# hjmkt/wrenc

Measured on AMD Instinct MI355X. Metric: all-intra encode fps at fixed QP (CTU RD search + final pass); bit-exactness vs the CPU oracle is checked in `parity`, higher is better.
Workload: dtype u8/i16/i32 (+i64 trellis costs, f32 RD cost)

## Files before the change

include/wrenc_gpu.h:

```cpp
#ifndef WRENC_GPU_H
#define WRENC_GPU_H

#include <stddef.h>
#include <stdint.h>

#ifdef __cplusplus
extern "C" {
#endif

typedef struct wrenc_gpu_ctx wrenc_gpu_ctx;

enum wrenc_gpu_status {
    WRENC_GPU_OK = 0,
    WRENC_GPU_EINVAL = -1,
    WRENC_GPU_ENODEV = -2,
    WRENC_GPU_ENOMEM = -3,
    WRENC_GPU_EHIP = -4,
    WRENC_GPU_ESTATE = -5,
    WRENC_GPU_ELEVEL = -6
};

typedef struct wrenc_gpu_config {
    int32_t width;
    int32_t height;
// ... 113 lines not shown
int wrenc_gpu_test_avail_tab(wrenc_gpu_ctx* ctx, int* differences);

int wrenc_gpu_stats_enable(wrenc_gpu_ctx* ctx, int on);

int wrenc_gpu_last_encode_stats(wrenc_gpu_ctx* ctx, float* total_ms, float* kernel_ms_sum,
                                int* n_launches);
typedef struct wrenc_gpu_kernel_stats {
    float ms_sum;
    int32_t launches;
    int64_t ctu_pictures;
} wrenc_gpu_kernel_stats;
int wrenc_gpu_last_encode_kernel_stats(wrenc_gpu_ctx* ctx, wrenc_gpu_kernel_stats out[2]);

int wrenc_gpu_final_pass_mismatches(wrenc_gpu_ctx* ctx, long long* count);

int wrenc_gpu_test_fwd_dct(wrenc_gpu_ctx* ctx, const int16_t* res, int log2n, int count,
                           int16_t* coef);
int wrenc_gpu_test_fwd_dct32(wrenc_gpu_ctx* ctx, const int16_t* res, int count, int16_t* coef,
                             int use_mfma, int reps, float* kernel_ms);
int wrenc_gpu_test_inv_dct32(wrenc_gpu_ctx* ctx, const int16_t* deq, int count, int16_t* res,
                             int use_mfma, int reps, float* kernel_ms);
int wrenc_gpu_test_quantize_pk(wrenc_gpu_ctx* ctx, const int16_t* coef, int log2n, int nc, int n_packs, int16_t* levels,
                               int64_t* level_cost);
int wrenc_gpu_test_inv_dct(wrenc_gpu_ctx* ctx, const int16_t* deq, int log2n, int count,
                           int16_t* res);
int wrenc_gpu_test_quantize(wrenc_gpu_ctx* ctx, const int16_t* coef, int log2n, int count,
                            int16_t* levels, int64_t* level_cost);
int wrenc_gpu_test_quantize_p16(wrenc_gpu_ctx* ctx, const int16_t* coef, int count, int16_t* levels,
                                int64_t* level_cost);
int wrenc_gpu_test_dequantize(wrenc_gpu_ctx* ctx, const int16_t* levels, int log2n, int count,
                              int16_t* deq);
int wrenc_gpu_test_fwd_dct4_reg(wrenc_gpu_ctx* ctx, const int16_t* res, int count, int16_t* coef);
int wrenc_gpu_test_inv_dct4_reg(wrenc_gpu_ctx* ctx, const int16_t* levels, int count, int16_t* res);

int wrenc_gpu_test_predict(wrenc_gpu_ctx* ctx, const uint8_t* rec_y, const uint8_t* rec_cb,
                           const uint8_t* rec_cr, int n_items, const int32_t* items, uint8_t* out,
                           size_t out_bytes);

#ifdef __cplusplus
}
#endif
#endif
```

wrenc_amd/csrc/dev_predict.h:

```cpp
#pragma once

namespace wrenc {

__device__ __forceinline__ int pdpc_w(int n_scale, int i) {
    const int sh = (i << 1) >> n_scale;
    return sh > 5 ? 0 : (32 >> sh);
}

__device__ __forceinline__ void build_refs(Ctx c, int comp, int tx, int ty, int tlg) {
#ifdef WRENC_EXP_SKIP_REFS
    return;
#endif
    c = uni(c);
    comp = uni(comp);
    tx = uni(tx);
    ty = uni(ty);
    tlg = uni(tlg);
    const int cs = comp ? 1 : 0;
    const int nb = comp ? 2 : 1;
    const int n = 1 << (tlg - cs);
    const int tn = 1 << tlg;
    const int cx = tx >> cs, cy = ty >> cs;
    const int st = 1 << cs;
    const int avm = block_avail_mask(c, tx, ty, tlg, st);
// ... 221 lines not shown
}
__device__ __forceinline__ void stage_org(const Ctx& c, int comps, int tx, int ty, int tlg, int lbyte = kOrgStage,
                                          int cword = 256) {
    uint32_t* dst = (uint32_t*)((char*)SH.r2 + lbyte);
#ifdef WRENC_EXP_NO_ORG
    for (int w = LANE; w < 384; w += 64) dst[w] = 0x50607080u + (uint32_t)w;
    WSYNC();
    return;
#endif
    if (comps & 1) {
        const int words = 1 << (2 * tlg - 2);
        for (int w = LANE; w < words; w += 64) {
            const int row = (4 * w) >> tlg, col = (4 * w) & ((1 << tlg) - 1);
            dst[w] = *(const GLOBAL_AS uint32_t*)&c.org[(ty + row) * 32 + tx + col];
        }
    }
    if (comps & 2) {
        const int lg = tlg - 1;
        const int words = 1 << (2 * lg - 2);
        for (int w = LANE; w < 2 * words; w += 64) {
            const int pl = w >= words ? 1 : 0;
            const int ww = w - pl * words;
            const int row = (4 * ww) >> lg, col = (4 * ww) & ((1 << lg) - 1);
            dst[cword + w] = *(const GLOBAL_AS uint32_t*)&c.org[1024 + pl * 256 + ((ty >> 1) + row) * 16 + (tx >> 1) + col];
        }
    }
    WSYNC();
}

__device__ __forceinline__ void stage_org_leaf(const Ctx& c, int comps, int tx, int ty, int tlg) {
    stage_org(c, comps, tx, ty, tlg, kOrgLeaf, 64);
}

enum { PRED_SCRATCH = 0, PRED_TILE = 1, PRED_PARK = 2, PRED_PARK16 = 3 };
constexpr int kParkByte = 160;
static_assert(kParkByte >= 144 && kParkByte % 16 == 0 && kParkByte + 288 <= 448, "Lds::decw: decisions of an 8x8 pack | its park | the server's results");
__device__ __forceinline__ uint8_t* park16(int i, int nl) {
    if (i < nl) return (uint8_t*)SH.r1 + 1536 + i;
    const int j = i - nl;
    return j < 128 ? (uint8_t*)SH.r2 + 1536 + j : (uint8_t*)SH.decw + 384 + (j - 128);
}
template <bool full>
__device__ __forceinline__ int emit_sample(const Ctx& c, int o, int i, int v, int pc, int x, int y, int to_tile, int nl = 0) {
    const int d = o - v;
    if (full) {
        SH.r1[i] = (int16_t)d;
        if (to_tile == PRED_TILE)
            rec_put(pc, x, y, v);
        else if (to_tile == PRED_PARK)
            ((uint8_t*)SH.decw)[kParkByte + i] = (uint8_t)v;
        else if (to_tile == PRED_PARK16)
            *park16(i, nl) = (uint8_t)v;
        else
            c.pred_scratch[i] = (uint8_t)v;
    }
    return d < 0 ? -d : d;
}

template <bool full>
__device__ __forceinline__ int predict(Ctx c, int comp, int tx, int ty, int tlg, int mode, int rbase = 0,
                                       int to_tile = PRED_TILE, int nl = 0, CclmPick pick = CclmPick{}) {
#ifdef WRENC_EXP_SKIP_PRED
    return 0;
#endif
    c = uni(c);
    rbase = uni(rbase);
    to_tile = uni(to_tile);
    nl = uni(nl);
    comp = uni(comp);
    tx = uni(tx);
    ty = uni(ty);
    tlg = uni(tlg);
    mode = uni(mode);
    const int cs = comp ? 1 : 0;
    const int nb = comp ? 2 : 1;
    const int lg = tlg - cs;
    const int n = 1 << lg;
    const int cx = tx >> cs, cy = ty >> cs;
    const int nn = n * n;
    const int obyte = org_byte(comp, tlg);
    const bool olds = tlg <= 4;
    int sad = 0;
    if (mode >= LT_CCLM) {
        CclmPick cp = pick;
        if (!pick.have) cp = cclm_pick(cclm_params(c, tx, ty, tlg, mode), 0);
        const int a0 = cp.a0, a1 = cp.a1, k0 = cp.k0, k1 = cp.k1, b0 = cp.b0, b1 = cp.b1;
        const bool flat128 = cp.flat128, avail_l = cp.avail_l;
// ... 589 lines not shown
```

wrenc_amd/csrc/dev_quant.h:

```cpp
#pragma once

namespace wrenc {

__device__ __forceinline__ long long ldq_at(Ctx c, int bits) {
    return bits < 256 ? (long long)SHT.ldq[bits] : c.k->ldq[bits];
}
__device__ __forceinline__ long long lv_at(Ctx c, int a) {
    return a < 256 ? (long long)SHT.lv[a] : c.k->lv[a];
}
template <int CTRL>
__device__ __forceinline__ int dpp_quad(int v) {
    return __builtin_amdgcn_mov_dpp(v, CTRL, 0xF, 0xF, true);
}

struct DecMasks {
    uint32_t m01, m23;
};
__device__ __forceinline__ DecMasks dec_masks(const uint16_t* dec16, int p) {
    const uint2 v = *(const uint2*)(dec16 + (p >> 4) * 4);
    DecMasks m;
    m.m01 = v.x;
    m.m23 = v.y;
    return m;
}
// ... 489 lines not shown
    unsigned zmask = 0;
    int fnz = P;
    int level = 0;
    if (mine) {
        int state = entry;
        level = (int16_t)emit_level(c, tc, qd, p == P - 1, nib, p, 0, state, zmask, sum_nz, fnz, ovf);
    }
    level = __builtin_amdgcn_ds_permute(4 * at, level);
    const int pf = row_min_i32(fnz);
    if (mine && (zmask & 1u) && p > pf) sum_nz += SHT.lv[0];
    {
        const long long hi = sum_nz >> 24;
        const int ra = row_sum_i32((int)(sum_nz & 0xFFFFFF)), rb = row_sum_i32((int)(hi & 0xFFFFFF)), rc = row_sum_i32((int)(hi >> 24));
#pragma unroll
        for (int b = 0; b < 4; ++b) {
            const long long a0 = (long long)(unsigned)__builtin_amdgcn_readlane(ra, 16 * b);
            const long long a1 = (long long)(unsigned)__builtin_amdgcn_readlane(rb, 16 * b);
            const long long a2 = (long long)__builtin_amdgcn_readlane(rc, 16 * b);
            lvl[b] = a0 + ((a1 + (a2 << 24)) << 24);
            if (__builtin_amdgcn_readlane(pf, 16 * b) < P) *any_mask |= 1 << b;
        }
    }
    if (__ballot(ovf != 0) != 0ULL) *overflow = 1;
    WSYNC();
    PROF_MARK(q3_);
    PROF_ADD2(PH_QTRACE, q2_, q3_);
    return level;
}
__device__ __forceinline__ int dequantize4_lane(const Ctx& c, int level) {
    constexpr int sh = 8 + 2 - 5 + 1, off = (1 << sh) >> 1;
    const int v = (M24(level, c.k->lsc) + off) >> sh;
    return min(max(v, -32768), 32767);
}


__device__ __forceinline__ void trace_rows64(const Ctx& c, int nblk, const int16_t* tcs, const uint16_t* dec16, int rbase,
                                             const CONST_AS uint16_t* scan, int sh, int off, long long lvl[4], bool any[4], int& ovf,
                                             int start = 0) {
    const int lane = lane_fresh();
    const int row = lane >> 4, i16 = lane & 15;
    const CONST_AS DevConst* k = c.k;
    const int per = start >= 48 ? 1 : (start >= 32 ? 2 : 4);
    const int p0 = start + i16 * per;
    const bool act = row < nblk && p0 < 64;
    const int b = row < nblk ? row : 0;
    const int16_t* btcs = tcs + b * 64;
    const DecMasks dm = dec_masks(dec16 + b * 16, act ? p0 : 0);
    int fmap = kMapId;
    if (act) {
        for (int j = 0; j < per; ++j) {
            const int p = p0 + j;
            const int tc = btcs[p];
            fmap = compose_map(position_map(tc, quotient(k, tc, sh, off), p == 63, dec_nib(dm, p)), fmap);
        }
    }
    int pre = fmap;
    pre = compose_map(pre, __builtin_amdgcn_update_dpp(kMapId, pre, 0x111, 0xF, 0xF, false));
    pre = compose_map(pre, __builtin_amdgcn_update_dpp(kMapId, pre, 0x112, 0xF, 0xF, false));
    pre = compose_map(pre, __builtin_amdgcn_update_dpp(kMapId, pre, 0x114, 0xF, 0xF, false));
    pre = compose_map(pre, __builtin_amdgcn_update_dpp(kMapId, pre, 0x118, 0xF, 0xF, false));
    int entry = __builtin_amdgcn_update_dpp(0, pre, 0x111, 0xF, 0xF, false) & 3;
    if (i16 == 0) entry = 0;
    long long sum_nz = 0;
    unsigned zmask = 0;
    int fnz = 64;
    if (act) {
// ... 419 lines not shown
```

wrenc_amd/csrc/dev_search.h:

```cpp
#pragma once

namespace wrenc {

enum { K_SADLIST = 0, K_FULL = 1, K_NOP = 2, K_SADSEARCH = 3, K_CCLMSEARCH = 4, K_SERVE8 = 5, K_LEAF8 = 7, K_LEAF16 = 8, K_SPLIT8 = 9, K_SERVE4 = 10 };
enum { COPY_NONE = 0, COPY_SAVE = 1, COPY_RESTORE = 2, COPY_PULL = 3 };

#if defined(WRENC_TRACE) || defined(WRENC_EXHAUSTIVE_SPLITS)
constexpr bool kSplitCut = false;
#else
constexpr bool kSplitCut = true;
#endif

#if defined(WRENC_TRACE) || defined(WRENC_EXHAUSTIVE_CANDIDATES)
constexpr bool kCandidateCut = false;
#else
constexpr bool kCandidateCut = true;
#endif

struct Req {
    int kind;
    int comps;
    int tx, ty, tlg;
    int ml, mc;
    bool active;
// ... 822 lines not shown
    if (c.trace && lane == 0) {
        TRACE_REC(c.ctu_x + q.tx, c.ctu_y + q.ty, 3, q.tree, 3, 0, cm, __float_as_int(c0));
        TRACE_REC(c.ctu_x + q.tx, c.ctu_y + q.ty, 3, q.tree, 3, 0, dm, __float_as_int(dm_cost));
    }
    const bool dm_wins = dm_keeps(dm_cost, c0);
    if ((row >= 2) == dm_wins) rec_put(1 + pl, (q.tx >> 1) + x, (q.ty >> 1) + y, p.rec);
    WSYNC();
    r.vmin = dm_wins ? dm_cost : c0;
    r.imin = dm_wins ? dm : cm;
    return r;
}

struct Pack8Out {
    uint32_t ssd_y[3], ssd_c[3];
    long long lvl_y[3], lvl_c[3];
};
template <class P>
__device__ __forceinline__ EvalParts pack_parts(const P& p, int k) {
    EvalParts e;
    e.ssd_y = p.ssd_y[k];
    e.ssd_c = p.ssd_c[k];
    e.lvl_y = p.lvl_y[k];
    e.lvl_c = p.lvl_c[k];
    return e;
}
__device__ __forceinline__ Pack8Out pack8_eval(const Ctx& c, const Req& q, int nc, int m0, int m1, int m2, int* overflow) {
    Pack8Out o;
    const int lane = lane_fresh();
    const int row = lane >> 4, i16 = lane & 15;
    const int nL = 64 * nc;
    uint8_t* park = (uint8_t*)SH.decw + kParkByte;
    const uint8_t* org = (const uint8_t*)SH.r2 + kOrgLeaf;
    PROF_MARK(t0_);
#pragma unroll 1
    for (int cd = 0; cd < nc; ++cd) {
        const int mode = cd == 0 ? m0 : (cd == 1 ? m1 : m2);
        if (mode != kNoMode) {
            predict<true>(c, 0, q.tx, q.ty, 3, mode, 64 * cd, PRED_PARK);
        } else {
            SH.r1[64 * cd + lane] = 0;
            park[64 * cd + lane] = 0;
        }
    }
#pragma unroll 1
    for (int ps = 0; ps < 2; ++ps) {
        if (4 * ps >= 2 * nc) continue;
        const int blk = 4 * ps + row;
        const int cd = blk >> 1, pl = blk & 1;
        const int mode = cd == 0 ? m0 : (cd == 1 ? m1 : m2);
        const bool in = blk < 2 * nc;
        const bool on = in && mode != kNoMode;
        const int v = predict4_lane(c, on ? mode : kNoMode, pl);
        int rc = on ? (int)org[256 + 16 * pl + i16] - v : 0;
        rc = fwd_dct4_reg(rc);
        if (in) {
            SH.r1[nL + 16 * blk + i16] = (int16_t)rc;
            park[nL + 16 * blk + i16] = (uint8_t)v;
        }
        WSYNC();
    }
    PROF_MARK(t1_);
    PROF_ADD2(PH_PREDICT, t0_, t1_);
    fwd_dct_lg(c, 3, nc, 0);
    PROF_MARK(t2_);
    PROF_ADD2(PH_FDCT, t1_, t2_);
    bool any_y = false, any_c = false;
    quantize_pk<3>(c, nc, overflow, o.lvl_y, o.lvl_c, &any_y, &any_c);
    PROF_MARK(t3_);
    if (any_y) {
        dequantize_t(c, 3, nc, 0);
        inv_dct_lg(c, 3, nc, 0);
    }
    PROF_MARK(t4_);
    PROF_ADD2(PH_IDCT, t3_, t4_);
#pragma unroll
    for (int cd = 0; cd < 3; ++cd) {
        o.ssd_y[cd] = 0;
        o.ssd_c[cd] = 0;
        if (cd < nc) {
            int rec = (int16_t)((int)park[64 * cd + lane] + (int)SH.r1[64 * cd + lane]);
            rec = min(max(rec, 0), 255);
            park[64 * cd + lane] = (uint8_t)rec;
            const int d = rec - (int)org[lane];
            o.ssd_y[cd] = (uint32_t)wave_sum_i32(M24(d, d));
        }
    }
#pragma unroll
    for (int ps = 0; ps < 2; ++ps) {
        if (4 * ps >= 2 * nc) continue;
        const int blk = 4 * ps + row;
        const bool in = blk < 2 * nc;
        int dd = 0;
        const int res = residual4_reg(c, in ? (int)SH.r1[nL + 16 * blk + i16] : 0, any_c);
        if (in) {
            int rec = (int16_t)((int)park[nL + 16 * blk + i16] + res);
            rec = min(max(rec, 0), 255);
            park[nL + 16 * blk + i16] = (uint8_t)rec;
            const int d = rec - (int)org[256 + 16 * (blk & 1) + i16];
            dd = M24(d, d);
        }
        const int rs = row_sum_i32(dd);
        const uint32_t s01 = (uint32_t)(__builtin_amdgcn_readlane(rs, 0) + __builtin_amdgcn_readlane(rs, 16));
        const uint32_t s23 = (uint32_t)(__builtin_amdgcn_readlane(rs, 32) + __builtin_amdgcn_readlane(rs, 48));
        if (ps == 0) {
            o.ssd_c[0] = s01;
            o.ssd_c[1] = s23;
        } else {
            o.ssd_c[2] = s01;
        }
    }
    WSYNC();
    PROF_MARK(t5_);
    PROF_ADD2(PH_RECON, t4_, t5_);
// ... 117 lines not shown
    r.imin2 = f.mc;
    return r;
}

__device__ __forceinline__ void serve_pack8(const Ctx& c, const Req& q, int* overflow) {
    const int lane = lane_fresh();
    const Lds& own = team_lds(c, 2);
    for (int w = lane; w < 98; w += 64) ((uint32_t*)SH.refs)[w] = ((const uint32_t*)own.refs)[w];
    for (int w = lane; w < 96; w += 64) ((uint32_t*)SH.r2)[kOrgLeaf / 4 + w] = ((const uint32_t*)own.r2)[kOrgLeaf / 4 + w];
    WSYNC();
    const Pack8Out a = pack8_eval(c, q, 2, PLANAR, DC, kNoMode, overflow);
    if (lane < 2) {
        XRes x;
        x.ssd_y = lane ? a.ssd_y[1] : a.ssd_y[0];
        x.ssd_c = lane ? a.ssd_c[1] : a.ssd_c[0];
        x.lvl_y = lane ? a.lvl_y[1] : a.lvl_y[0];
        x.lvl_c = lane ? a.lvl_c[1] : a.lvl_c[0];
        SH.xr[lane] = x;
    }
    WSYNC();
    lv_word_add(&SHT.lvb.job_done);
}

struct Pack16Out {
    uint32_t ssd_y[2], ssd_c[2];
    long long lvl_y[3], lvl_c[3];
};
__device__ __forceinline__ Pack16Out pack16_eval(const Ctx& c, const Req& q, int nc, int m0, int m1, int* overflow) {
    Pack16Out o;
    const int lane = lane_fresh();
    const int nL = 256 * nc;
    const uint8_t* org = (const uint8_t*)SH.r2 + kOrgLeaf;
    PROF_MARK(t0_);
#pragma unroll 1
    for (int cd = 0; cd < nc; ++cd) {
        const int mode = cd == 0 ? m0 : m1;
        if (mode != kNoMode) {
            predict<true>(c, 0, q.tx, q.ty, 4, mode, 256 * cd, PRED_PARK16, nL);
            predict<true>(c, 1, q.tx, q.ty, 4, mode, nL + 128 * cd, PRED_PARK16, nL);
        } else {
            for (int i = lane; i < 256; i += 64) {
                SH.r1[256 * cd + i] = 0;
                *park16(256 * cd + i, nL) = 0;
            }
            for (int i = lane; i < 128; i += 64) {
                SH.r1[nL + 128 * cd + i] = 0;
                *park16(nL + 128 * cd + i, nL) = 0;
            }
            WSYNC();
        }
    }
    PROF_MARK(t1_);
    PROF_ADD2(PH_PREDICT, t0_, t1_);
    fwd_dct_lg(c, 4, nc, 0);
    fwd_dct_lg(c, 3, 2 * nc, nL);
    PROF_MARK(t2_);
    PROF_ADD2(PH_FDCT, t1_, t2_);
    bool any_y = false, any_c = false;
    quantize_pk<4>(c, nc, overflow, o.lvl_y, o.lvl_c, &any_y, &any_c);
    PROF_MARK(t3_);
    if (any_y) {
        dequantize_t(c, 4, nc, 0);
        inv_dct_lg(c, 4, nc, 0);
    }
    if (any_c) {
        dequantize_t(c, 3, 2 * nc, nL);
        inv_dct_lg(c, 3, 2 * nc, nL);
    }
    PROF_MARK(t4_);
    PROF_ADD2(PH_IDCT, t3_, t4_);
#pragma unroll
    for (int cd = 0; cd < 2; ++cd) {
        o.ssd_y[cd] = 0;
        o.ssd_c[cd] = 0;
        if (cd < nc) {
            int py = 0, pc = 0;
#pragma unroll
            for (int kq = 0; kq < 4; ++kq) {
                const int i = lane + 64 * kq;
                uint8_t* pk = park16(256 * cd + i, nL);
                int rec = (int16_t)((int)*pk + (int)SH.r1[256 * cd + i]);
                rec = min(max(rec, 0), 255);
                *pk = (uint8_t)rec;
                const int d = rec - (int)org[i];
                py += M24(d, d);
            }
#pragma unroll
            for (int kq = 0; kq < 2; ++kq) {
                const int i = lane + 64 * kq;
                uint8_t* pk = park16(nL + 128 * cd + i, nL);
                int rec = (int16_t)((int)*pk + (int)SH.r1[nL + 128 * cd + i]);
                rec = min(max(rec, 0), 255);
                *pk = (uint8_t)rec;
                const int d = rec - (int)org[256 + i];
                pc += M24(d, d);
            }
            o.ssd_y[cd] = (uint32_t)wave_sum_i32(py);
            o.ssd_c[cd] = (uint32_t)wave_sum_i32(pc);
        }
    }
    WSYNC();
    PROF_MARK(t5_);
    PROF_ADD2(PH_RECON, t4_, t5_);
    return o;
}

__device__ __forceinline__ void pack16_to_tile(const Ctx& c, const Req& q, int nc, int cd) {
    const int lane = lane_fresh();
#pragma unroll
    for (int kq = 0; kq < 4; ++kq) {
        const int i = lane + 64 * kq;
        rec_put(0, q.tx + (i & 15), q.ty + (i >> 4), *park16(256 * cd + i, 256 * nc));
    }
#pragma unroll
    for (int kq = 0; kq < 2; ++kq) {
        const int i = lane + 64 * kq;
        rec_put(1 + (i >> 6), (q.tx >> 1) + (i & 7), (q.ty >> 1) + ((i & 63) >> 3), *park16(256 * nc + 128 * cd + i, 256 * nc));
    }
    WSYNC();
}

__device__ __forceinline__ Res leaf16_search(const Ctx& c, const Req& q, int* overflow) {
    Res r = res_none();
    const int lane = lane_fresh();
// ... 1245 lines not shown
```

wrenc_amd/csrc/dev_transform.h:

```cpp
#pragma once

namespace wrenc {

__device__ __forceinline__ int dot2(uint32_t a, uint32_t b, int acc) {
    typedef short s2 __attribute__((ext_vector_type(2)));
    s2 va, vb;
    va.x = (short)(a & 0xFFFF);
    va.y = (short)(a >> 16);
    vb.x = (short)(b & 0xFFFF);
    vb.y = (short)(b >> 16);
    return __builtin_amdgcn_sdot2(va, vb, acc, false);
}

template <int LG, int HBYTES>
__device__ void fwd_dct(Ctx c, int nb, int o1, LDS_AS int32_t* h) {
    constexpr int N = 1 << LG;
    constexpr int G = 64 / N;
    constexpr int HS = N + 1;
    const int u = LANE & (N - 1);
    const int g = LANE >> LG;
    uint32_t t[N / 2];
    {
        const CONST_AS uint32_t* src = (const CONST_AS uint32_t*)&c.k->dct[LG - 2][u][0];
#pragma unroll
// ... 199 lines not shown
    constexpr uint32_t w = t4_word(STAGE, K);
    return (int)(int8_t)(w >> shift8);
}
template <int STAGE, bool QUAD>
__device__ __forceinline__ int t4_stage(int v, int shift8) {
    const int v0 = QUAD ? dpp_mov<0x00>(v) : v;
    const int v1 = QUAD ? dpp_mov<0x55>(v) : dpp_mov<0x124>(v);
    const int v2 = QUAD ? dpp_mov<0xAA>(v) : dpp_mov<0x128>(v);
    const int v3 = QUAD ? dpp_mov<0xFF>(v) : dpp_mov<0x12C>(v);
    const int t0 = t4_sel<STAGE, 0>(shift8), t1 = t4_sel<STAGE, 1>(shift8), t2 = t4_sel<STAGE, 2>(shift8), t3 = t4_sel<STAGE, 3>(shift8);
    const int acc = M24(v0, t0) + M24(v1, t1) + M24(v2, t2) + M24(v3, t3);
    return acc;
}

__device__ __forceinline__ int fwd_dct4_reg(int res) {
#ifdef WRENC_EXP_SKIP_DCT
    return res;
#endif
    const int lane = lane_fresh();
    const int sx = 8 * (lane & 3), sy = 2 * (lane & 12);
    const int h = (t4_stage<T4_FWD1, true>(res, sx) + 1) >> 1;
    return (int16_t)((t4_stage<T4_FWD2, false>(h, sy) + 128) >> 8);
}

__device__ __forceinline__ int inv_dct4_reg(int deq) {
#ifdef WRENC_EXP_SKIP_DCT
    return deq;
#endif
    const int lane = lane_fresh();
    const int sx = 8 * (lane & 3), sy = 2 * (lane & 12);
    int v = (t4_stage<T4_INV1, false>(deq, sy) + 64) >> 7;
    v = min(max(v, -32768), 32767);
    return (int16_t)((t4_stage<T4_INV2, true>(v, sx) + 2048) >> 12);
}

__device__ __forceinline__ void fwd_dct_lg(Ctx c, int lg, int nb, int o1 = 0) {
#ifdef WRENC_EXP_SKIP_DCT
    return;
#endif
    c = uni(c);
    lg = uni(lg);
    nb = uni(nb);
    o1 = uni(o1);
    LDS_AS int32_t* h = (LDS_AS int32_t*)SH.r2;
    constexpr int HB = (int)sizeof(SH.r2);
    switch (lg) {
    case 2: fwd_dct<2, HB>(c, nb, o1, h); break;
    case 3: fwd_dct<3, HB>(c, nb, o1, h); break;
    case 4: fwd_dct<4, HB>(c, nb, o1, h); break;
    default:
        fwd_dct32_mfma(c, o1);
        break;
    }
}
__device__ __forceinline__ void inv_dct_lg(Ctx c, int lg, int nb, int o1 = 0) {
#ifdef WRENC_EXP_SKIP_DCT
    return;
#endif
    c = uni(c);
    lg = uni(lg);
    nb = uni(nb);
    o1 = uni(o1);
    switch (lg) {
    case 2: inv_dct<2>(c, nb, o1); break;
    case 3: inv_dct<3>(c, nb, o1); break;
    case 4: inv_dct<4>(c, nb, o1); break;
// ... 12 lines not shown
```

wrenc_amd/csrc/wrenc_gpu.hip:

```cpp
#include "../../include/wrenc_gpu.h"
#include "wrenc_dev.h"

#include <hip/hip_runtime.h>

#include <cmath>
#include <cstdio>
#include <cstring>
#include <new>
#include <string>
#include <vector>

using namespace wrenc;

constexpr int kXcdMax = 8;
constexpr int kRegionsPerXcd = 256;
constexpr int kAffineRegions = kXcdMax * kRegionsPerXcd;
constexpr int kOverflowRegions = 2048;
constexpr int kScratchSlots = kAffineRegions + kOverflowRegions;
constexpr int kSlotMapWords = kScratchSlots / 64 + 1;

__device__ __forceinline__ int xcc_id() {
    return (int)(__builtin_amdgcn_s_getreg(20 | (0 << 6) | ((4 - 1) << 11)) & (kXcdMax - 1));
}
__device__ __forceinline__ int take_region(unsigned long long* slot_map, unsigned w0, unsigned nw) {
// ... 299 lines not shown
    if (above_right_avail(c, bx, by, lg) != (((m >> 4) & 1) != 0)) atomicAdd(out, 1);
    if (below_left_avail(c, bx, by, lg) != ((m & 1) != 0)) atomicAdd(out, 1);
    if (nb_avail(c, gx, gy, tn, gx - 1, gy, false, false) != (((m >> 1) & 1) != 0)) atomicAdd(out, 1);
    if (nb_avail(c, gx, gy, tn, gx, gy - 1, false, false) != (((m >> 3) & 1) != 0)) atomicAdd(out, 1);
}

__global__ __launch_bounds__(64) void test_quantize_p16_kernel(const DevConst* __restrict__ k, const int16_t* in, int count,
                                                               int16_t* out, long long* cost, int* overflow) {
    Ctx c = {};
    c.k = (const CONST_AS DevConst*)k;
    load_tables(c);
    const int first = 4 * blockIdx.x;
    const int nb = min(4, count - first);
    const bool mine = threadIdx.x < 16 * nb;
    int ovf = 0, any = 0;
    long long lvl[4];
    const int level = quantize_p16_reg(c, nb, mine ? (int)in[(size_t)first * 16 + threadIdx.x] : 0, &ovf, lvl, &any);
    if (mine) out[(size_t)first * 16 + threadIdx.x] = (int16_t)level;
    if (threadIdx.x == 0) {
        for (int b = 0; b < nb; ++b) cost[first + b] = lvl[b];
        if (ovf) atomicOr(overflow, 1);
    }
}

__global__ __launch_bounds__(64) void test_dct4_reg_kernel(const DevConst* __restrict__ k, const int16_t* in, int count, int inverse,
                                                           int16_t* out) {
    Ctx c = {};
    c.k = (const CONST_AS DevConst*)k;
    const size_t at = (size_t)blockIdx.x * 64 + threadIdx.x;
    const bool mine = at < (size_t)count * 16;
    const int v = mine ? (int)in[at] : 0;
    const int r = inverse ? inv_dct4_reg(dequantize4_lane(c, v)) : fwd_dct4_reg(v);
    if (mine) out[at] = (int16_t)r;
}

__global__ __launch_bounds__(64) void test_quantize_pk_kernel(const DevConst* __restrict__ k, const int16_t* in, int lgl, int nc,
                                                              int16_t* out, long long* cost, int* overflow) {
    Ctx c = {};
    c.k = (const CONST_AS DevConst*)k;
    load_tables(c);
    const int total = nc * 3 * (1 << (2 * lgl)) / 2;
    for (int i = threadIdx.x; i < total; i += 64) SH.r1[i] = in[(size_t)blockIdx.x * total + i];
    WSYNC();
    int ovf = 0;
    bool any_y = false, any_c = false;
    long long ly[3], lc[3];
    if (lgl == 3)
        quantize_pk<3>(c, nc, &ovf, ly, lc, &any_y, &any_c);
    else
        quantize_pk<4>(c, nc, &ovf, ly, lc, &any_y, &any_c);
    for (int i = threadIdx.x; i < total; i += 64) out[(size_t)blockIdx.x * total + i] = SH.r1[i];
    if (threadIdx.x == 0) {
        for (int b = 0; b < nc; ++b) {
            cost[((size_t)blockIdx.x * nc + b) * 2] = ly[b];
            cost[((size_t)blockIdx.x * nc + b) * 2 + 1] = lc[b];
        }
        if (ovf) atomicOr(overflow, 1);
    }
}

__global__ __launch_bounds__(64) void test_dequantize_kernel(const DevConst* __restrict__ k,
                                                             const int16_t* in, int lg, int16_t* out) {
    Ctx c = {};
    c.k = (const CONST_AS DevConst*)k;
    const int n = 1 << lg, nn = n * n;
    for (int i = threadIdx.x; i < nn; i += 64) SH.r1[i] = in[(size_t)blockIdx.x * nn + i];
// ... 1687 lines not shown
    if (e == hipSuccess) e = hipEventElapsedTime(&ms, e0, e1);
    if (e == hipSuccess) e = hipMemcpy(out, d_out, bytes, hipMemcpyDeviceToHost);
    if (kernel_ms) *kernel_ms = ms;
    (void)hipFree(d_in);
    if (d_out) (void)hipFree(d_out);
    if (e0) (void)hipEventDestroy(e0);
    if (e1) (void)hipEventDestroy(e1);
    if (e != hipSuccess) return fail(ctx, WRENC_GPU_EHIP, hipGetErrorString(e));
    return WRENC_GPU_OK;
}
int wrenc_gpu_test_fwd_dct32(wrenc_gpu_ctx* ctx, const int16_t* res, int count, int16_t* coef, int use_mfma, int reps,
                             float* kernel_ms) {
    return run_dct32_bench(ctx, res, count, coef, use_mfma, reps, kernel_ms, false);
}
int wrenc_gpu_test_inv_dct32(wrenc_gpu_ctx* ctx, const int16_t* deq, int count, int16_t* res, int use_mfma, int reps,
                             float* kernel_ms) {
    return run_dct32_bench(ctx, deq, count, res, use_mfma, reps, kernel_ms, true);
}
int wrenc_gpu_test_inv_dct(wrenc_gpu_ctx* ctx, const int16_t* deq, int log2n, int count, int16_t* res) {
    return run_block_test(ctx, deq, log2n, count, res, [&](int16_t* i, int16_t* o) {
        hipLaunchKernelGGL(test_inv_dct_kernel, dim3(count), dim3(64), 0, ctx->stream, ctx->d_const, i, log2n, o);
    });
}
int wrenc_gpu_test_fwd_dct4_reg(wrenc_gpu_ctx* ctx, const int16_t* res, int count, int16_t* coef) {
    return run_block_test(ctx, res, 2, count, coef, [&](int16_t* i, int16_t* o) {
        hipLaunchKernelGGL(test_dct4_reg_kernel, dim3((count + 3) / 4), dim3(64), 0, ctx->stream, ctx->d_const, i, count, 0, o);
    });
}
int wrenc_gpu_test_inv_dct4_reg(wrenc_gpu_ctx* ctx, const int16_t* levels, int count, int16_t* res) {
    return run_block_test(ctx, levels, 2, count, res, [&](int16_t* i, int16_t* o) {
        hipLaunchKernelGGL(test_dct4_reg_kernel, dim3((count + 3) / 4), dim3(64), 0, ctx->stream, ctx->d_const, i, count, 1, o);
    });
}
int wrenc_gpu_test_dequantize(wrenc_gpu_ctx* ctx, const int16_t* levels, int log2n, int count, int16_t* deq) {
    return run_block_test(ctx, levels, log2n, count, deq, [&](int16_t* i, int16_t* o) {
        hipLaunchKernelGGL(test_dequantize_kernel, dim3(count), dim3(64), 0, ctx->stream, ctx->d_const, i, log2n, o);
    });
}
int wrenc_gpu_test_quantize(wrenc_gpu_ctx* ctx, const int16_t* coef, int log2n, int count, int16_t* levels,
                            int64_t* level_cost) {
    if (!ctx || !level_cost) return WRENC_GPU_EINVAL;
    if (count < 1) return fail(ctx, WRENC_GPU_EINVAL, "count must be >= 1");
    HIP_TRY(ctx, hipSetDevice(ctx->cfg.device));
    long long* d_cost = nullptr;
    HIP_TRY(ctx, hipMalloc((void**)&d_cost, sizeof(long long) * count));
    int rc = run_block_test(ctx, coef, log2n, count, levels, [&](int16_t* i, int16_t* o) {
        hipLaunchKernelGGL(test_quantize_kernel, dim3(count), dim3(64), 0, ctx->stream, ctx->d_const, i, log2n, o,
                           d_cost, ctx->d_overflow + 1);
    });
    if (rc == WRENC_GPU_OK) {
        hipError_t e = hipMemcpy(level_cost, d_cost, sizeof(long long) * count, hipMemcpyDeviceToHost);
        if (e != hipSuccess) rc = fail(ctx, WRENC_GPU_EHIP, hipGetErrorString(e));
    }
    (void)hipFree(d_cost);
    return take_test_overflow(ctx, rc);
}

int wrenc_gpu_test_quantize_p16(wrenc_gpu_ctx* ctx, const int16_t* coef, int count, int16_t* levels, int64_t* level_cost) {
    if (!ctx || !level_cost) return WRENC_GPU_EINVAL;
    if (count < 1) return fail(ctx, WRENC_GPU_EINVAL, "count must be >= 1");
    HIP_TRY(ctx, hipSetDevice(ctx->cfg.device));
    long long* d_cost = nullptr;
    HIP_TRY(ctx, hipMalloc((void**)&d_cost, sizeof(long long) * count));
    int rc = run_block_test(ctx, coef, 2, count, levels, [&](int16_t* i, int16_t* o) {
        hipLaunchKernelGGL(test_quantize_p16_kernel, dim3((count + 3) / 4), dim3(64), 0, ctx->stream, ctx->d_const, i, count, o,
                           d_cost, ctx->d_overflow + 1);
// ... 88 lines not shown
```

wrenc_amd/gpu.py:

```python
import ctypes as C
import os

import numpy as np

os.environ.setdefault("GPU_MAX_HW_QUEUES", "8")

_HERE = os.path.dirname(os.path.abspath(__file__))
LIB_PATH = os.environ.get("WRENC_GPU_LIB", os.path.join(_HERE, "csrc", "libwrenc_gpu.so"))

EXPORTED_SYMBOLS = [
    "wrenc_gpu_default_config", "wrenc_gpu_config_extra_params", "wrenc_gpu_create", "wrenc_gpu_destroy", "wrenc_gpu_last_error",
    "wrenc_gpu_upload", "wrenc_gpu_encode", "wrenc_gpu_set_slot_qp", "wrenc_gpu_sync", "wrenc_gpu_download", "wrenc_gpu_download_compact", "wrenc_gpu_compact_mask_words", "wrenc_gpu_expand_levels", "wrenc_gpu_download_tokens", "wrenc_gpu_download_metrics", "wrenc_gpu_download_complexity", "wrenc_gpu_metrics_values", "wrenc_gpu_test_metrics", "wrenc_gpu_test_load_record", "wrenc_gpu_device_info",
    "wrenc_gpu_alloc_host", "wrenc_gpu_free_host", "wrenc_gpu_encode_picture", "wrenc_gpu_set_schedule", "wrenc_gpu_last_schedule", "wrenc_gpu_stats_enable", "wrenc_gpu_last_encode_stats", "wrenc_gpu_last_encode_kernel_stats", "wrenc_gpu_final_pass_mismatches",
    "wrenc_gpu_test_fwd_dct", "wrenc_gpu_test_inv_dct", "wrenc_gpu_test_quantize",
    "wrenc_gpu_test_dequantize", "wrenc_gpu_test_predict", "wrenc_gpu_test_fwd_dct32", "wrenc_gpu_test_inv_dct32", "wrenc_gpu_test_quantize_p16", "wrenc_gpu_test_quantize_pk", "wrenc_gpu_test_fwd_dct4_reg", "wrenc_gpu_test_inv_dct4_reg", "wrenc_gpu_test_set_wave_slots", "wrenc_gpu_test_scratch_overflows", "wrenc_gpu_test_head_ranges", "wrenc_gpu_test_avail_tab",
    "wrenc_gpu_set_visible_size", "wrenc_gpu_visible_size", "wrenc_gpu_test_download_originals",
]


class Config(C.Structure):
    _fields_ = [
        ("width", C.c_int32), ("height", C.c_int32), ("qp", C.c_int32), ("max_split_depth", C.c_int32),
        ("device", C.c_int32), ("n_slots", C.c_int32),
        ("lv_table", C.c_int64 * 1024), ("dq_table", C.c_int64 * 1024),
        ("lambda_q", C.c_int64), ("lambda_rd", C.c_float), ("lambda_rd_chroma", C.c_float),
        ("header_bits_luma", C.c_int64 * 67 * 4 * 2),
        ("header_bits_chroma", C.c_int64 * 4),
    ]


class Picture(C.Structure):
    _fields_ = [
        ("rec_y", C.c_void_p), ("rec_cb", C.c_void_p), ("rec_cr", C.c_void_p),
        ("lev_y", C.c_void_p), ("lev_cb", C.c_void_p), ("lev_cr", C.c_void_p),
        ("cu_log2_size", C.c_void_p), ("luma_mode", C.c_void_p), ("chroma_mode", C.c_void_p),
        ("ctu_cost", C.c_void_p),
    ]


class Compact(C.Structure):
    _fields_ = [("mask", C.c_void_p), ("payload", C.c_void_p), ("payload_cap", C.c_size_t), ("n_blocks", C.c_size_t),
                ("cu_log2_size", C.c_void_p), ("luma_mode", C.c_void_p), ("chroma_mode", C.c_void_p),
                ("rec_y", C.c_void_p), ("rec_cb", C.c_void_p), ("rec_cr", C.c_void_p)]


class Tokens(C.Structure):
    _fields_ = [("first_page", C.c_void_p), ("cu_log2_size", C.c_void_p), ("luma_mode", C.c_void_p), ("chroma_mode", C.c_void_p),
                ("rec_y", C.c_void_p), ("rec_cb", C.c_void_p), ("rec_cr", C.c_void_p)]
# ... 387 lines not shown
        return out

    def fwd_dct(self, blocks):
        return self._blocks(self.lib.wrenc_gpu_test_fwd_dct, blocks)

    def fwd_dct32(self, blocks, use_mfma, reps=1):
        arr = np.ascontiguousarray(blocks, np.int16)
        assert arr.shape[1:] == (32, 32)
        out = np.zeros_like(arr)
        ms = C.c_float()
        self.lib.wrenc_gpu_test_fwd_dct32.argtypes = [C.c_void_p, C.c_void_p, C.c_int, C.c_void_p, C.c_int, C.c_int,
                                                      C.POINTER(C.c_float)]
        self._check(self.lib.wrenc_gpu_test_fwd_dct32(self.ctx, _p(arr), arr.shape[0], _p(out), int(use_mfma), int(reps),
                                                      C.byref(ms)))
        return out, ms.value

    def inv_dct32(self, blocks, use_mfma, reps=1):
        arr = np.ascontiguousarray(blocks, np.int16)
        assert arr.shape[1:] == (32, 32)
        out = np.zeros_like(arr)
        ms = C.c_float()
        self.lib.wrenc_gpu_test_inv_dct32.argtypes = [C.c_void_p, C.c_void_p, C.c_int, C.c_void_p, C.c_int, C.c_int,
                                                      C.POINTER(C.c_float)]
        self._check(self.lib.wrenc_gpu_test_inv_dct32(self.ctx, _p(arr), arr.shape[0], _p(out), int(use_mfma), int(reps),
                                                      C.byref(ms)))
        return out, ms.value

    def inv_dct(self, blocks):
        return self._blocks(self.lib.wrenc_gpu_test_inv_dct, blocks)

    def dequantize(self, blocks):
        return self._blocks(self.lib.wrenc_gpu_test_dequantize, blocks)

    def _blocks4_reg(self, fn, blocks):
        arr = np.ascontiguousarray(blocks, np.int16)
        assert arr.shape[1:] == (4, 4)
        out = np.zeros_like(arr)
        fn.argtypes = [C.c_void_p, C.c_void_p, C.c_int, C.c_void_p]
        self._check(fn(self.ctx, _p(arr), arr.shape[0], _p(out)))
        return out

    def fwd_dct4_reg(self, blocks):
        return self._blocks4_reg(self.lib.wrenc_gpu_test_fwd_dct4_reg, blocks)

    def inv_dct4_reg(self, levels):
        return self._blocks4_reg(self.lib.wrenc_gpu_test_inv_dct4_reg, levels)

    def predict_blocks(self, rec_y, rec_cb, rec_cr, items):
        items = np.ascontiguousarray(items, np.int32).reshape(-1, 5)
        sizes = [((1 << int(q[2])) ** 2) // (2 if q[3] == 1 else 1) for q in items]
        out = np.zeros(int(sum(sizes)), np.uint8)
        planes = [np.ascontiguousarray(a, np.uint8) for a in (rec_y, rec_cb, rec_cr)]
        assert planes[0].shape == (self.height, self.width)
        self.lib.wrenc_gpu_test_predict.argtypes = [C.c_void_p, C.c_void_p, C.c_void_p, C.c_void_p, C.c_int, C.c_void_p,
                                                    C.c_void_p, C.c_size_t]
        self._check(self.lib.wrenc_gpu_test_predict(self.ctx, _p(planes[0]), _p(planes[1]), _p(planes[2]), len(items),
                                                    _p(items), _p(out), out.size))
        res, at = [], 0
        for q, sz in zip(items, sizes):
            n = 1 << int(q[2])
            blk = out[at:at + sz]
            res.append(blk.reshape(2, n // 2, n // 2) if q[3] == 1 else blk.reshape(n, n))
            at += sz
        return res

    def sad_lists(self, rec_y, rec_cb, rec_cr, items):
        it = np.ascontiguousarray(items, np.int32).reshape(-1, 7)
        dev = np.zeros((len(it), 5), np.int32)
        dev[:, :3] = it[:, :3]
        dev[:, 3] = np.where(it[:, 3] == 4, 7, 3 + it[:, 3])
        dev[:, 4] = np.where(it[:, 3] == 4, 0, it[:, 4] | (it[:, 5] << 8) | (it[:, 6] << 16))
        out = np.zeros(64 * len(it), np.uint8)
        planes = [np.ascontiguousarray(a, np.uint8) for a in (rec_y, rec_cb, rec_cr)]
        assert planes[0].shape == (self.height, self.width)
        self.lib.wrenc_gpu_test_predict.argtypes = [C.c_void_p, C.c_void_p, C.c_void_p, C.c_void_p, C.c_int, C.c_void_p,
                                                    C.c_void_p, C.c_size_t]
        self._check(self.lib.wrenc_gpu_test_predict(self.ctx, _p(planes[0]), _p(planes[1]), _p(planes[2]), len(dev),
                                                    _p(dev), _p(out), out.size))
        return out.view(np.uint32).reshape(len(it), 16)
# ... 30 lines not shown
```

Before: 226.5.

## Compute 8x8 DCT/IDCT in registers via DPP and bpermute for leaf packs

```diff
diff --git a/include/wrenc_gpu.h b/include/wrenc_gpu.h
--- a/include/wrenc_gpu.h
+++ b/include/wrenc_gpu.h
@@ -169,6 +169,8 @@
                               int16_t* deq);
 int wrenc_gpu_test_fwd_dct4_reg(wrenc_gpu_ctx* ctx, const int16_t* res, int count, int16_t* coef);
 int wrenc_gpu_test_inv_dct4_reg(wrenc_gpu_ctx* ctx, const int16_t* levels, int count, int16_t* res);
+int wrenc_gpu_test_fwd_dct8_reg(wrenc_gpu_ctx* ctx, const int16_t* res, int count, int16_t* coef);
+int wrenc_gpu_test_inv_dct8_reg(wrenc_gpu_ctx* ctx, const int16_t* levels, int count, int16_t* res);
 
 int wrenc_gpu_test_predict(wrenc_gpu_ctx* ctx, const uint8_t* rec_y, const uint8_t* rec_cb,
                            const uint8_t* rec_cr, int n_items, const int32_t* items, uint8_t* out,
diff --git a/wrenc_amd/csrc/dev_predict.h b/wrenc_amd/csrc/dev_predict.h
--- a/wrenc_amd/csrc/dev_predict.h
+++ b/wrenc_amd/csrc/dev_predict.h
@@ -277,7 +277,7 @@
     stage_org(c, comps, tx, ty, tlg, kOrgLeaf, 64);
 }
 
-enum { PRED_SCRATCH = 0, PRED_TILE = 1, PRED_PARK = 2, PRED_PARK16 = 3 };
+enum { PRED_SCRATCH = 0, PRED_TILE = 1, PRED_PARK = 2, PRED_PARK16 = 3, PRED_PARK_REG = 4, PRED_PARK16_REG = 5 };
 constexpr int kParkByte = 160;
 static_assert(kParkByte >= 144 && kParkByte % 16 == 0 && kParkByte + 288 <= 448, "Lds::decw: decisions of an 8x8 pack | its park | the server's results");
 __device__ __forceinline__ uint8_t* park16(int i, int nl) {
@@ -289,15 +289,17 @@
 __device__ __forceinline__ int emit_sample(const Ctx& c, int o, int i, int v, int pc, int x, int y, int to_tile, int nl = 0) {
     const int d = o - v;
     if (full) {
-        SH.r1[i] = (int16_t)d;
+        const bool reg = to_tile == PRED_PARK_REG || to_tile == PRED_PARK16_REG;
+        if (!reg) SH.r1[i] = (int16_t)d;
         if (to_tile == PRED_TILE)
             rec_put(pc, x, y, v);
-        else if (to_tile == PRED_PARK)
+        else if (to_tile == PRED_PARK || to_tile == PRED_PARK_REG)
             ((uint8_t*)SH.decw)[kParkByte + i] = (uint8_t)v;
-        else if (to_tile == PRED_PARK16)
+        else if (to_tile == PRED_PARK16 || to_tile == PRED_PARK16_REG)
             *park16(i, nl) = (uint8_t)v;
         else
             c.pred_scratch[i] = (uint8_t)v;
+        if (reg) return (int)((uint32_t)(d & 0xFFFF) << (pc == 2 ? 16 : 0));
     }
     return d < 0 ? -d : d;
 }
diff --git a/wrenc_amd/csrc/dev_quant.h b/wrenc_amd/csrc/dev_quant.h
--- a/wrenc_amd/csrc/dev_quant.h
+++ b/wrenc_amd/csrc/dev_quant.h
@@ -545,6 +545,11 @@
     const int v = (M24(level, c.k->lsc) + off) >> sh;
     return min(max(v, -32768), 32767);
 }
+__device__ __forceinline__ int dequantize8_lane(const Ctx& c, int level) {
+    constexpr int sh = 8 + 3 - 5 + 1, off = (1 << sh) >> 1;
+    const int v = (M24(level, c.k->lsc) + off) >> sh;
+    return min(max(v, -32768), 32767);
+}
 
 
 __device__ __forceinline__ void trace_rows64(const Ctx& c, int nblk, const int16_t* tcs, const uint16_t* dec16, int rbase,
diff --git a/wrenc_amd/csrc/dev_search.h b/wrenc_amd/csrc/dev_search.h
--- a/wrenc_amd/csrc/dev_search.h
+++ b/wrenc_amd/csrc/dev_search.h
@@ -878,15 +878,14 @@
     uint8_t* park = (uint8_t*)SH.decw + kParkByte;
     const uint8_t* org = (const uint8_t*)SH.r2 + kOrgLeaf;
     PROF_MARK(t0_);
+    int resy = 0;
 #pragma unroll 1
     for (int cd = 0; cd < nc; ++cd) {
         const int mode = cd == 0 ? m0 : (cd == 1 ? m1 : m2);
-        if (mode != kNoMode) {
-            predict<true>(c, 0, q.tx, q.ty, 3, mode, 64 * cd, PRED_PARK);
-        } else {
-            SH.r1[64 * cd + lane] = 0;
+        if (mode != kNoMode)
+            resy |= (predict<true>(c, 0, q.tx, q.ty, 3, mode, 64 * cd, PRED_PARK_REG) & 0x3FF) << (10 * cd);
+        else
             park[64 * cd + lane] = 0;
-        }
     }
 #pragma unroll 1
     for (int ps = 0; ps < 2; ++ps) {
@@ -907,15 +906,21 @@
     }
     PROF_MARK(t1_);
     PROF_ADD2(PH_PREDICT, t0_, t1_);
-    fwd_dct_lg(c, 3, nc, 0);
+    const int cidx = dct8_reg_index(lane);
+#pragma unroll
+    for (int cd = 0; cd < 3; ++cd)
+        if (cd < nc) SH.r1[64 * cd + cidx] = (int16_t)fwd_dct8_reg((int)((uint32_t)resy << (22 - 10 * cd)) >> 22);
+    WSYNC();
     PROF_MARK(t2_);
     PROF_ADD2(PH_FDCT, t1_, t2_);
     bool any_y = false, any_c = false;
     quantize_pk<3>(c, nc, overflow, o.lvl_y, o.lvl_c, &any_y, &any_c);
     PROF_MARK(t3_);
+    int res[3] = {0, 0, 0};
     if (any_y) {
-        dequantize_t(c, 3, nc, 0);
-        inv_dct_lg(c, 3, nc, 0);
+#pragma unroll
+        for (int cd = 0; cd < 3; ++cd)
+            if (cd < nc) res[cd] = inv_dct8_reg(dequantize8_lane(c, SH.r1[64 * cd + cidx]));
     }
     PROF_MARK(t4_);
     PROF_ADD2(PH_IDCT, t3_, t4_);
@@ -924,7 +929,7 @@
         o.ssd_y[cd] = 0;
         o.ssd_c[cd] = 0;
         if (cd < nc) {
-            int rec = (int16_t)((int)park[64 * cd + lane] + (int)SH.r1[64 * cd + lane]);
+            int rec = (int16_t)((int)park[64 * cd + lane] + res[cd]);
             rec = min(max(rec, 0), 255);
             park[64 * cd + lane] = (uint8_t)rec;
             const int d = rec - (int)org[lane];
@@ -1108,28 +1113,38 @@
     const int nL = 256 * nc;
     const uint8_t* org = (const uint8_t*)SH.r2 + kOrgLeaf;
     PROF_MARK(t0_);
+    int rc0 = 0, rc1 = 0;
 #pragma unroll 1
     for (int cd = 0; cd < nc; ++cd) {
         const int mode = cd == 0 ? m0 : m1;
         if (mode != kNoMode) {
             predict<true>(c, 0, q.tx, q.ty, 4, mode, 256 * cd, PRED_PARK16, nL);
-            predict<true>(c, 1, q.tx, q.ty, 4, mode, nL + 128 * cd, PRED_PARK16, nL);
+            const int d = predict<true>(c, 1, q.tx, q.ty, 4, mode, nL + 128 * cd, PRED_PARK16_REG, nL);
+            if (cd == 0)
+                rc0 = d;
+            else
+                rc1 = d;
         } else {
             for (int i = lane; i < 256; i += 64) {
                 SH.r1[256 * cd + i] = 0;
                 *park16(256 * cd + i, nL) = 0;
             }
-            for (int i = lane; i < 128; i += 64) {
-                SH.r1[nL + 128 * cd + i] = 0;
-                *park16(nL + 128 * cd + i, nL) = 0;
-            }
+            for (int i = lane; i < 128; i += 64) *park16(nL + 128 * cd + i, nL) = 0;
             WSYNC();
         }
     }
     PROF_MARK(t1_);
     PROF_ADD2(PH_PREDICT, t0_, t1_);
+    const int cidx = dct8_reg_index(lane);
+#pragma unroll
+    for (int cd = 0; cd < 2; ++cd)
+        if (cd < nc) {
+            const int d = cd ? rc1 : rc0;
+            SH.r1[nL + 128 * cd + cidx] = (int16_t)fwd_dct8_reg((int)(int16_t)d);
+            SH.r1[nL + 128 * cd + 64 + cidx] = (int16_t)fwd_dct8_reg(d >> 16);
+        }
+    WSYNC();
     fwd_dct_lg(c, 4, nc, 0);
-    fwd_dct_lg(c, 3, 2 * nc, nL);
     PROF_MARK(t2_);
     PROF_ADD2(PH_FDCT, t1_, t2_);
     bool any_y = false, any_c = false;
@@ -1139,9 +1154,14 @@
         dequantize_t(c, 4, nc, 0);
         inv_dct_lg(c, 4, nc, 0);
     }
+    int resc[2][2] = {{0, 0}, {0, 0}};
     if (any_c) {
-        dequantize_t(c, 3, 2 * nc, nL);
-        inv_dct_lg(c, 3, 2 * nc, nL);
+#pragma unroll
+        for (int cd = 0; cd < 2; ++cd)
+            if (cd < nc) {
+                resc[cd][0] = inv_dct8_reg(dequantize8_lane(c, SH.r1[nL + 128 * cd + cidx]));
+                resc[cd][1] = inv_dct8_reg(dequantize8_lane(c, SH.r1[nL + 128 * cd + 64 + cidx]));
+            }
     }
     PROF_MARK(t4_);
     PROF_ADD2(PH_IDCT, t3_, t4_);
@@ -1165,7 +1185,7 @@
             for (int kq = 0; kq < 2; ++kq) {
                 const int i = lane + 64 * kq;
                 uint8_t* pk = park16(nL + 128 * cd + i, nL);
-                int rec = (int16_t)((int)*pk + (int)SH.r1[nL + 128 * cd + i]);
+                int rec = (int16_t)((int)*pk + resc[cd][kq]);
                 rec = min(max(rec, 0), 255);
                 *pk = (uint8_t)rec;
                 const int d = rec - (int)org[256 + i];
diff --git a/wrenc_amd/csrc/dev_transform.h b/wrenc_amd/csrc/dev_transform.h
--- a/wrenc_amd/csrc/dev_transform.h
+++ b/wrenc_amd/csrc/dev_transform.h
@@ -255,6 +255,76 @@
     int v = (t4_stage<T4_INV1, false>(deq, sy) + 64) >> 7;
     v = min(max(v, -32768), 32767);
     return (int16_t)((t4_stage<T4_INV2, true>(v, sx) + 2048) >> 12);
+}
+
+constexpr int kT8[8][8] = {{64, 64, 64, 64, 64, 64, 64, 64},     {89, 75, 50, 18, -18, -50, -75, -89},
+                           {83, 36, -36, -83, -83, -36, 36, 83}, {75, -18, -89, -50, 50, 89, 18, -75},
+                           {64, -64, -64, 64, 64, -64, -64, 64}, {50, -89, 18, 75, -75, -18, 89, -50},
+                           {36, -83, 83, -36, -36, 83, -83, 36}, {18, -50, 75, -89, 89, -75, 50, -18}};
+constexpr int t8_freq(int p) { return ((p << 1) & 6) | (p >> 2); }
+enum { T8_FWD, T8_INV };
+constexpr uint32_t t8_word(int dir, int k, int half) {
+    uint32_t w = 0;
+    for (int j = 0; j < 4; ++j) {
+        const int p = 4 * half + j;
+        const int t = dir == T8_FWD ? (p < 4 ? kT8[2 * p][k] : -kT8[2 * p - 7][3 - k])
+                                    : (p < 4 ? kT8[2 * k][p] : kT8[2 * k + 1][7 - p]);
+        w |= (uint32_t)(t & 0xFF) << (8 * j);
+    }
+    return w;
+}
+template <int DIR, int K>
+__device__ __forceinline__ int t8_sel(bool odd, int shift8) {
+    constexpr uint32_t w0 = t8_word(DIR, K, 0), w1 = t8_word(DIR, K, 1);
+    return (int)(int8_t)((odd ? w1 : w0) >> shift8);
+}
+struct T8Basis {
+    int t0, t1, t2, t3;
+};
+template <int DIR>
+__device__ __forceinline__ T8Basis t8_basis(int lane) {
+    const bool odd = (lane & 4) != 0;
+    const int s8 = 8 * (lane & 3);
+    return T8Basis{t8_sel<DIR, 0>(odd, s8), t8_sel<DIR, 1>(odd, s8), t8_sel<DIR, 2>(odd, s8), t8_sel<DIR, 3>(odd, s8)};
+}
+__device__ __forceinline__ int t8_quad_sum(int v, const T8Basis& t) {
+    return M24(dpp_mov<0x00>(v), t.t0) + M24(dpp_mov<0x55>(v), t.t1) + M24(dpp_mov<0xAA>(v), t.t2) + M24(dpp_mov<0xFF>(v), t.t3);
+}
+__device__ __forceinline__ int t8_fwd_stage(int v, const T8Basis& t, bool odd) {
+    const int m = dpp_mov<kDppRowHalfMirror>(v);
+    return t8_quad_sum(odd ? v - m : v + m, t);
+}
+__device__ __forceinline__ int t8_inv_stage(int v, const T8Basis& t, bool odd) {
+    const int e = t8_quad_sum(v, t);
+    const int m = dpp_mov<kDppRowHalfMirror>(e);
+    return odd ? m - e : e + m;
+}
+__device__ __forceinline__ int dct8_reg_index(int lane) { return 8 * t8_freq(lane & 7) + (lane >> 3); }
+
+__device__ __forceinline__ int fwd_dct8_reg(int res) {
+#ifdef WRENC_EXP_SKIP_DCT
+    return res;
+#endif
+    const int lane = lane_fresh();
+    const bool odd = (lane & 4) != 0;
+    const T8Basis t = t8_basis<T8_FWD>(lane);
+    int h = (t8_fwd_stage(res, t, odd) + 2) >> 2;
+    const int a = lane >> 3, b = lane & 7;
+    h = __builtin_amdgcn_ds_bpermute(4 * (8 * b + ((a >> 1) | ((a & 1) << 2))), h);
+    return (int16_t)((t8_fwd_stage(h, t, odd) + 256) >> 9);
+}
+
+__device__ __forceinline__ int inv_dct8_reg(int deq) {
+#ifdef WRENC_EXP_SKIP_DCT
+    return deq;
+#endif
+    const int lane = lane_fresh();
+    const bool odd = (lane & 4) != 0;
+    const T8Basis t = t8_basis<T8_INV>(lane);
+    int v = (t8_inv_stage(deq, t, odd) + 64) >> 7;
+    v = min(max(v, -32768), 32767);
+    v = __builtin_amdgcn_ds_bpermute(4 * (8 * t8_freq(lane & 7) + (lane >> 3)), v);
+    return (int16_t)((t8_inv_stage(v, t, odd) + 2048) >> 12);
 }
 
 __device__ __forceinline__ void fwd_dct_lg(Ctx c, int lg, int nb, int o1 = 0) {
diff --git a/wrenc_amd/csrc/wrenc_gpu.hip b/wrenc_amd/csrc/wrenc_gpu.hip
--- a/wrenc_amd/csrc/wrenc_gpu.hip
+++ b/wrenc_amd/csrc/wrenc_gpu.hip
@@ -355,6 +355,17 @@
     const int v = mine ? (int)in[at] : 0;
     const int r = inverse ? inv_dct4_reg(dequantize4_lane(c, v)) : fwd_dct4_reg(v);
     if (mine) out[at] = (int16_t)r;
+}
+
+__global__ __launch_bounds__(64) void test_dct8_reg_kernel(const DevConst* __restrict__ k, const int16_t* in, int inverse, int16_t* out) {
+    Ctx c = {};
+    c.k = (const CONST_AS DevConst*)k;
+    const size_t base = (size_t)blockIdx.x * 64;
+    const int lane = (int)threadIdx.x, cidx = dct8_reg_index(lane);
+    if (inverse)
+        out[base + lane] = (int16_t)inv_dct8_reg(dequantize8_lane(c, in[base + cidx]));
+    else
+        out[base + cidx] = (int16_t)fwd_dct8_reg(in[base + lane]);
 }
 
 __global__ __launch_bounds__(64) void test_quantize_pk_kernel(const DevConst* __restrict__ k, const int16_t* in, int lgl, int nc,
@@ -2108,6 +2119,16 @@
         hipLaunchKernelGGL(test_dct4_reg_kernel, dim3((count + 3) / 4), dim3(64), 0, ctx->stream, ctx->d_const, i, count, 1, o);
     });
 }
+int wrenc_gpu_test_fwd_dct8_reg(wrenc_gpu_ctx* ctx, const int16_t* res, int count, int16_t* coef) {
+    return run_block_test(ctx, res, 3, count, coef, [&](int16_t* i, int16_t* o) {
+        hipLaunchKernelGGL(test_dct8_reg_kernel, dim3(count), dim3(64), 0, ctx->stream, ctx->d_const, i, 0, o);
+    });
+}
+int wrenc_gpu_test_inv_dct8_reg(wrenc_gpu_ctx* ctx, const int16_t* levels, int count, int16_t* res) {
+    return run_block_test(ctx, levels, 3, count, res, [&](int16_t* i, int16_t* o) {
+        hipLaunchKernelGGL(test_dct8_reg_kernel, dim3(count), dim3(64), 0, ctx->stream, ctx->d_const, i, 1, o);
+    });
+}
 int wrenc_gpu_test_dequantize(wrenc_gpu_ctx* ctx, const int16_t* levels, int log2n, int count, int16_t* deq) {
     return run_block_test(ctx, levels, log2n, count, deq, [&](int16_t* i, int16_t* o) {
         hipLaunchKernelGGL(test_dequantize_kernel, dim3(count), dim3(64), 0, ctx->stream, ctx->d_const, i, log2n, o);
diff --git a/wrenc_amd/gpu.py b/wrenc_amd/gpu.py
--- a/wrenc_amd/gpu.py
+++ b/wrenc_amd/gpu.py
@@ -13,7 +13,7 @@
     "wrenc_gpu_upload", "wrenc_gpu_encode", "wrenc_gpu_set_slot_qp", "wrenc_gpu_sync", "wrenc_gpu_download", "wrenc_gpu_download_compact", "wrenc_gpu_compact_mask_words", "wrenc_gpu_expand_levels", "wrenc_gpu_download_tokens", "wrenc_gpu_download_metrics", "wrenc_gpu_download_complexity", "wrenc_gpu_metrics_values", "wrenc_gpu_test_metrics", "wrenc_gpu_test_load_record", "wrenc_gpu_device_info",
     "wrenc_gpu_alloc_host", "wrenc_gpu_free_host", "wrenc_gpu_encode_picture", "wrenc_gpu_set_schedule", "wrenc_gpu_last_schedule", "wrenc_gpu_stats_enable", "wrenc_gpu_last_encode_stats", "wrenc_gpu_last_encode_kernel_stats", "wrenc_gpu_final_pass_mismatches",
     "wrenc_gpu_test_fwd_dct", "wrenc_gpu_test_inv_dct", "wrenc_gpu_test_quantize",
-    "wrenc_gpu_test_dequantize", "wrenc_gpu_test_predict", "wrenc_gpu_test_fwd_dct32", "wrenc_gpu_test_inv_dct32", "wrenc_gpu_test_quantize_p16", "wrenc_gpu_test_quantize_pk", "wrenc_gpu_test_fwd_dct4_reg", "wrenc_gpu_test_inv_dct4_reg", "wrenc_gpu_test_set_wave_slots", "wrenc_gpu_test_scratch_overflows", "wrenc_gpu_test_head_ranges", "wrenc_gpu_test_avail_tab",
+    "wrenc_gpu_test_dequantize", "wrenc_gpu_test_predict", "wrenc_gpu_test_fwd_dct32", "wrenc_gpu_test_inv_dct32", "wrenc_gpu_test_quantize_p16", "wrenc_gpu_test_quantize_pk", "wrenc_gpu_test_fwd_dct4_reg", "wrenc_gpu_test_inv_dct4_reg", "wrenc_gpu_test_fwd_dct8_reg", "wrenc_gpu_test_inv_dct8_reg", "wrenc_gpu_test_set_wave_slots", "wrenc_gpu_test_scratch_overflows", "wrenc_gpu_test_head_ranges", "wrenc_gpu_test_avail_tab",
     "wrenc_gpu_set_visible_size", "wrenc_gpu_visible_size", "wrenc_gpu_test_download_originals",
 ]
 
@@ -467,9 +467,9 @@
     def dequantize(self, blocks):
         return self._blocks(self.lib.wrenc_gpu_test_dequantize, blocks)
 
-    def _blocks4_reg(self, fn, blocks):
+    def _blocks4_reg(self, fn, blocks, n=4):
         arr = np.ascontiguousarray(blocks, np.int16)
-        assert arr.shape[1:] == (4, 4)
+        assert arr.shape[1:] == (n, n)
         out = np.zeros_like(arr)
         fn.argtypes = [C.c_void_p, C.c_void_p, C.c_int, C.c_void_p]
         self._check(fn(self.ctx, _p(arr), arr.shape[0], _p(out)))
@@ -480,6 +480,12 @@
 
     def inv_dct4_reg(self, levels):
         return self._blocks4_reg(self.lib.wrenc_gpu_test_inv_dct4_reg, levels)
+
+    def fwd_dct8_reg(self, blocks):
+        return self._blocks4_reg(self.lib.wrenc_gpu_test_fwd_dct8_reg, blocks, 8)
+
+    def inv_dct8_reg(self, levels):
+        return self._blocks4_reg(self.lib.wrenc_gpu_test_inv_dct8_reg, levels, 8)
 
     def predict_blocks(self, rec_y, rec_cb, rec_cr, items):
         items = np.ascontiguousarray(items, np.int32).reshape(-1, 5)
```

After: 227.7 (median of 6 runs). About the same (+0.6%).
